# theEricMa/ScaleDreamer

Measured on AMD Instinct MI355X. Metric: ASD train steps/sec (64x64 render, SD2.1), higher is better.
Workload: dtype f32 renderer / f16 diffusion (f32 accumulate); 1 GPU; asd_sd_nerf: 1 view/GPU, 64x64 rays, 512 spp occgrid march, implicit-volume iNGP (16x2 hash grid 2^19, MLP 64), SD-2.1 UNet batch 5 (CFG+Perp-Neg+shifted t), VAE 512^2 fwd+bwd, AdamW; views_per_gpu=1, parallelism=dp1, diffusion_backend=hip, diffusion_weights=seeded random init (seed 1)

## Files before the change

scaledreamer_amd/csrc/gemm.hip:

```cpp
#include <stdlib.h>

#include "asd_common.h"
#include <map>
#include <atomic>
#include <mutex>
#include <cstring>
#include <iterator>

#include "gemm_tile.h"


template <int BM, int BN, int WM, int WN, bool CONV, int NST = 2, int KG = 1, bool LN = false>
__global__ __launch_bounds__(WM * WN * KG * 64) void gemm_f16_kernel(const asd_gemm_args p) {
    constexpr int NW = WM * WN;
    constexpr int TM = BM / WM / 16, TN = BN / WN / 16;
    constexpr int RB = 128;
    constexpr int A_BYTES = BM * RB, B_BYTES = BN * RB;
    constexpr int STAGE_BYTES = A_BYTES + B_BYTES;
    constexpr int ASLABS = BM / 8, TSLABS = (BM + BN) / 8;
    constexpr int SPW = (TSLABS + NW - 1) / NW;
    static_assert(BM % (WM * 16) == 0 && BN % (WN * 16) == 0, "wave tile must be a multiple of 16 x 16");
    static_assert(NST == 2 || TSLABS % NW == 0, "ring variants count their loads per wave: every wave must own the same number of slabs");
    static_assert(KG == 1 || NST == 2, "k-groups use the two-stage loop");
    extern __shared__ __attribute__((aligned(16))) char smem[];

    const int tid = threadIdx.x, lane = tid & 63;
    const int wave_all = __builtin_amdgcn_readfirstlane(tid >> 6);
    const int kg = KG > 1 ? wave_all / NW : 0;
    const int wave = wave_all - kg * NW;
    char* const gsm = smem + kg * (NST * STAGE_BYTES);
    const int wm = wave / WN, wn = wave % WN;
    const bool up3 = CONV && p.upsample == 3;
    const int up_mq = up3 ? p.M >> 2 : 1;
    const int tiles_pp = (up_mq + BM - 1) / BM;
    const int tiles_m = up3 ? 4 * tiles_pp : (p.M + BM - 1) / BM, tiles_n = (p.N + BN - 1) / BN;
    int item, tm_, tn_;
    if (!asd_xcd_item(blockIdx.x, tiles_m * tiles_n * p.split_k, item)) return;
    const int kz = item / (tiles_m * tiles_n);
    asd_grouped_tile(item - kz * tiles_m * tiles_n, tiles_m, tiles_n, p.group_m, p.group_n, tm_, tn_);
    const int parity = up3 ? tm_ / tiles_pp : 0;
    const int m0 = up3 ? parity * up_mq + (tm_ - parity * tiles_pp) * BM : tm_ * BM, n0 = tn_ * BN;
    const int m_lim = up3 ? (parity + 1) * up_mq : p.M;
    const int k_steps_total = (p.K + 63) / 64;
    const int k_per = (k_steps_total + p.split_k - 1) / p.split_k;
    const int ks0 = kz * k_per, ks1 = min(k_steps_total, ks0 + k_per);

// ... 246 lines not shown
#pragma unroll
            for (int s = 0; s < NST - 1; ++s)
                if (s < nk) issue(ks0 + s, s);
            int stage = 0, fill = NST - 1;
            for (int i = 0; i < nk; ++i) {
                ring_wait<SPW, NST - 2>(nk - 1 - i);
                __builtin_amdgcn_s_barrier();
                if (i + NST - 1 < nk) issue(ks0 + i + NST - 1, fill);
                compute(gsm + stage * STAGE_BYTES);
                stage = stage + 1 == NST ? 0 : stage + 1;
                fill = fill + 1 == NST ? 0 : fill + 1;
            }
        }
    } else {
    int k = ks0;
    while (k < ks1 && !live(k)) ++k;
    if (k < ks1) {
        issue(k, 0);
        for (int stage = 0;; stage ^= 1) {
            asm volatile("s_waitcnt vmcnt(0)" ::: "memory");
            __builtin_amdgcn_s_barrier();
            int kn = k + 1;
            while (kn < ks1 && !live(kn)) ++kn;
            if (kn < ks1) issue(kn, stage ^ 1);
            compute(gsm + stage * STAGE_BYTES);
            if (kn >= ks1) break;
            k = kn;
        }
    }
    }
    if constexpr (KG == 1) ln_extract();

    const int em = lane & 15, en = (lane >> 4) * 4;
    auto out_row = [&](int i) {
        const int m = m0 + wm * (BM / WM) + i * 16 + em;
        if (m >= m_lim) return -1;
        if (CONV && p.upsample == 3) {
            const int q = m - parity * up_mq, hwq = p.Hin * p.Win;
            const int bb = q / hwq, r = q - bb * hwq, y = r / p.Win, x = r - y * p.Win;
            return (bb * p.Hout + 2 * y + par_a) * p.Wout + 2 * x + par_b;
        }
        return m;
    };
    if (KG > 1 && kg != 0) {
        if (p.split_k == 1 && p.act != 2 && p.gn_partials != nullptr) {
            __syncthreads(); __syncthreads();
            __syncthreads();
        }
        return;
    }
    if (p.split_k > 1) {
        tile_epilogue<TM, TN>(p, acc, n0 + wn * (BN / WN), kz, m0, out_row, false, nullptr);
        return;
    }
    float ln_mean[LN ? TM : 1], ln_rstd[LN ? TM : 1];
    if constexpr (LN) {
        const float inv_k = 1.f / (float)p.K;
#pragma unroll
        for (int i = 0; i < TM; ++i) {
            ln_mean[i] = ls1[i] * inv_k;
            ln_rstd[i] = rsqrtf(fmaxf(ls2[i] * inv_k - ln_mean[i] * ln_mean[i], 0.f) + p.ln_eps);
            const int m = m0 + wm * (BM / WM) + i * 16 + em;
            if (p.ln_stats && n0 == 0 && wn == 0 && lane < 16 && m < p.M) { p.ln_stats[2 * m] = ln_mean[i]; p.ln_stats[2 * m + 1] = ln_rstd[i]; }
        }
    }
    if (p.act == 2) {
        if constexpr (TN % 2 == 0) {
#pragma unroll
            for (int i = 0; i < TM; ++i) {
                const int m = m0 + wm * (BM / WM) + i * 16 + em;
                if (m >= p.M) continue;
#pragma unroll
                for (int j = 0; j < TN; j += 2) {
                    const int n = n0 + wn * (BN / WN) + j * 16 + en;
                    if (n + 16 >= p.N) continue;
                    const half4 bx = *(const half4*)((const half_t*)p.bias + n), bg = *(const half4*)((const half_t*)p.bias + n + 16);
                    float va[4] = {acc[i][j][0], acc[i][j][1], acc[i][j][2], acc[i][j][3]};
                    float vg[4] = {acc[i][j + 1][0], acc[i][j + 1][1], acc[i][j + 1][2], acc[i][j + 1][3]};
                    if (p.ln_mode) {
                        ln_fold<4>(p, va, m, n, LN ? ln_mean[i] : 0.f, LN ? ln_rstd[i] : 0.f);
                        ln_fold<4>(p, vg, m, n + 16, LN ? ln_mean[i] : 0.f, LN ? ln_rstd[i] : 0.f);
                    }
                    half4 o;
#pragma unroll
                    for (int r = 0; r < 4; ++r)
// ... 270 lines not shown
                            acc[i][j] = __builtin_amdgcn_mfma_f32_16x16x32_f16(wb[kh][j], xa[kh][i], acc[i][j], 0, 0, 0);
            } else {
#pragma unroll
            for (int kh = 0; kh < 2; ++kh) {
                half8 xa[TM], wb[TN];
                const char* Ak = Ar + (((kh * 4 + fq) ^ csw) * 16);
#pragma unroll
                for (int i = 0; i < TM; ++i) xa[i] = *(const half8*)(Ak + i * WIN * RB);
#pragma unroll
                for (int j = 0; j < TN; ++j) wb[j] = *(const half8*)(Wt + fb0 + fswb[kh] + j * 16 * RB);
#pragma unroll
                for (int i = 0; i < TM; ++i)
#pragma unroll
                    for (int j = 0; j < TN; ++j)
                        acc[i][j] = __builtin_amdgcn_mfma_f32_16x16x32_f16(wb[j], xa[i], acc[i][j], 0, 0, 0);
            }
            }
        }
    }

    const bool gn = p.gn_partials != nullptr && p.split_k == 1;
    float* gn_lds = (float*)smem;
    if (gn) gn_tile_begin(gn_lds);
    tile_epilogue<TM, TN>(p, acc, n0 + wn * (BN / WN), kz, b * p.Hout * p.Wout,
                          [&](int i) { return (b * p.Hout + y0 + wm * 4 + i) * p.Wout + x0 + frow; }, gn, gn_lds);
    if (gn) gn_tile_end(p, gn_lds, tm * tiles_n + tn_);
}

__global__ __launch_bounds__(256) void splitk_epilogue_kernel(const asd_gemm_args p, int splits) {
    const size_t q = (size_t)blockIdx.x * 256 + threadIdx.x;
    const size_t total4 = (size_t)p.M * p.N / 4;
    if (q >= total4) return;
    const int m = (int)((q * 4) / p.N), n = (int)((q * 4) % p.N);
    floatx4 v = {0.f, 0.f, 0.f, 0.f};
    for (int s = 0; s < splits; ++s) {
        const floatx4 t = *(const floatx4*)(p.workspace + ((size_t)s * p.M + m) * p.N + n);
        v[0] += t[0]; v[1] += t[1]; v[2] += t[2]; v[3] += t[3];
    }
    if (p.bias) {
        const half4 b = *(const half4*)((const half_t*)p.bias + n);
        v[0] += (float)b[0]; v[1] += (float)b[1]; v[2] += (float)b[2]; v[3] += (float)b[3];
    }
    if (p.row_bias) {
        const half4 b = *(const half4*)((const half_t*)p.row_bias + (size_t)(m / p.rows_per_group) * p.ld_row_bias + n);
        v[0] += (float)b[0]; v[1] += (float)b[1]; v[2] += (float)b[2]; v[3] += (float)b[3];
    }
    if (p.act == 1) {
#pragma unroll
        for (int r = 0; r < 4; ++r) v[r] = asd_silu_fast(v[r]);
    }
    if (p.residual) {
        const half4 b = *(const half4*)((const half_t*)p.residual + (size_t)m * p.ldr + n);
        v[0] += (float)b[0]; v[1] += (float)b[1]; v[2] += (float)b[2]; v[3] += (float)b[3];
    }
    if (p.out_f32) {
        *(floatx4*)((float*)p.C + (size_t)m * p.ldc + n) = v;
    } else {
        half4 o = {(half_t)v[0], (half_t)v[1], (half_t)v[2], (half_t)v[3]};
        *(half4*)((half_t*)p.C + (size_t)m * p.ldc + n) = o;
    }
}

__global__ __launch_bounds__(256) void splitk_epilogue_gn_kernel(const asd_gemm_args p, int splits) {
    __shared__ float lds64[64];
    const int tiles_n = p.N / 64;
    const int mb = blockIdx.x / tiles_n, nb = blockIdx.x - mb * tiles_n;
    const int tx = threadIdx.x & 15, ty = threadIdx.x >> 4;
    const int n = nb * 64 + tx * 4;
    if (threadIdx.x < 64) lds64[threadIdx.x] = 0.f;
    __syncthreads();
    floatx4 cs = {0.f, 0.f, 0.f, 0.f}, cq = {0.f, 0.f, 0.f, 0.f};
    half4 bias = {0, 0, 0, 0};
    if (p.bias) bias = *(const half4*)((const half_t*)p.bias + n);
    floatx4 v[4];
    int mrow[4];
#pragma unroll
    for (int i = 0; i < 4; ++i) {
        v[i] = floatx4{0.f, 0.f, 0.f, 0.f};
        mrow[i] = min(mb * 64 + i * 16 + ty, p.M - 1);
    }
    for (int s = 0; s < splits; ++s) {
        floatx4 t[4];
#pragma unroll
        for (int i = 0; i < 4; ++i) t[i] = *(const floatx4*)(p.workspace + ((size_t)s * p.M + mrow[i]) * p.N + n);
#pragma unroll
        for (int i = 0; i < 4; ++i) { v[i][0] += t[i][0]; v[i][1] += t[i][1]; v[i][2] += t[i][2]; v[i][3] += t[i][3]; }
    }
#pragma unroll
    for (int i = 0; i < 4; ++i) {
        const int m = mb * 64 + i * 16 + ty;
        if (m >= p.M) continue;
        floatx4 w = v[i];
        w[0] += (float)bias[0]; w[1] += (float)bias[1]; w[2] += (float)bias[2]; w[3] += (float)bias[3];
        if (p.row_bias) {
            const half4 b = *(const half4*)((const half_t*)p.row_bias + (size_t)(m / p.rows_per_group) * p.ld_row_bias + n);
            w[0] += (float)b[0]; w[1] += (float)b[1]; w[2] += (float)b[2]; w[3] += (float)b[3];
        }
        if (p.act == 1) {
#pragma unroll
            for (int r = 0; r < 4; ++r) w[r] = asd_silu_fast(w[r]);
        }
        if (p.residual) {
            const half4 b = *(const half4*)((const half_t*)p.residual + (size_t)m * p.ldr + n);
            w[0] += (float)b[0]; w[1] += (float)b[1]; w[2] += (float)b[2]; w[3] += (float)b[3];
        }
        const half4 o = {(half_t)w[0], (half_t)w[1], (half_t)w[2], (half_t)w[3]};
        *(half4*)((half_t*)p.C + (size_t)m * p.ldc + n) = o;
#pragma unroll
        for (int r = 0; r < 4; ++r) { const float f = (float)o[r]; cs[r] += f; cq[r] = fmaf(f, f, cq[r]); }
    }
#pragma unroll
    for (int r = 0; r < 4; ++r) {
        const int g = (n + r) / p.gn_cg;
        atomicAdd(&lds64[2 * g], cs[r]);
        atomicAdd(&lds64[2 * g + 1], cq[r]);
    }
    __syncthreads();
    if (threadIdx.x < 64) p.gn_partials[(size_t)blockIdx.x * 64 + threadIdx.x] = lds64[threadIdx.x];
}

#define GNA_THREADS 1024
template <int NV>
__global__ __launch_bounds__(GNA_THREADS) void splitk_epilogue_gnapply_kernel(const asd_gemm_args p, int splits, float inv_cnt ) {
    __shared__ float red[2 * (GNA_THREADS / 64)];
    const int cg = p.gn_cg, g4 = cg >> 2, rows = p.gn_rows;
    const int b = blockIdx.x >> 5, g = blockIdx.x & 31;
    const int n0 = g * cg, total = rows * g4, tid = threadIdx.x;
    floatx4 v[NV];
    int mrow[NV], ncol[NV];
#pragma unroll
    for (int i = 0; i < NV; ++i) {
        const int e = min(tid + GNA_THREADS * i, total - 1);
        const int r = e / g4;
        mrow[i] = b * rows + r;
        ncol[i] = n0 + (e - r * g4) * 4;
        v[i] = floatx4{0.f, 0.f, 0.f, 0.f};
    }
    half4 bias[NV], rbias[NV], resid[NV];
#pragma unroll
    for (int i = 0; i < NV; ++i) {
        const int m = mrow[i], n = ncol[i];
        bias[i] = p.bias ? *(const half4*)((const half_t*)p.bias + n) : half4{0, 0, 0, 0};
        rbias[i] = p.row_bias ? *(const half4*)((const half_t*)p.row_bias + (size_t)(m / p.rows_per_group) * p.ld_row_bias + n) : half4{0, 0, 0, 0};
        resid[i] = p.residual ? *(const half4*)((const half_t*)p.residual + (size_t)m * p.ldr + n) : half4{0, 0, 0, 0};
    }
    for (int s = 0; s < splits; s += 4) {
        floatx4 t[4][NV];
#pragma unroll
        for (int u = 0; u < 4; ++u) {
            const int su = min(s + u, splits - 1);
#pragma unroll
// ... 54 lines not shown
#pragma unroll
        for (int r = 0; r < 4; ++r) {
            const float sa = rstd * (float)gm[r];
            float f = fmaf(v[i][r], sa, (float)bt[r] - mean * sa);
            if (p.gn_apply_silu) f = asd_silu_fast(f);
            o[r] = (half_t)f;
        }
        *(half4*)((half_t*)p.gn_apply_y + (size_t)m * p.N + n) = o;
    }
}

static int asd_gemm_gn_apply_nv(const asd_gemm_args* a) {
    if (!a->gn_apply || a->split_k <= 1 || a->partials_only || a->out_f32 || a->act == 2 || a->gn_bwd_x) return 0;
    if (a->gn_cg < 4 || a->gn_cg % 4 || a->N != 32 * a->gn_cg || a->gn_rows < 1 || a->M % a->gn_rows || a->ldc % 4) return 0;
    if (a->conv && a->upsample == 3) return 0;
    const int need = (a->gn_rows * (a->gn_cg / 4) + GNA_THREADS - 1) / GNA_THREADS;
    return need <= 1 ? 1 : need <= 3 ? 3 : 0;
}

static void asd_launch_splitk_epilogue(const asd_gemm_args* a, hipStream_t s) {
    const int nv = a->gn_apply_y ? asd_gemm_gn_apply_nv(a) : 0;
    if (nv > 0) {
        const dim3 grid((a->M / a->gn_rows) * 32);
        const float inv_cnt = 1.f / ((float)a->gn_rows * (float)a->gn_cg);
        if (nv == 1) hipLaunchKernelGGL(splitk_epilogue_gnapply_kernel<1>, grid, dim3(GNA_THREADS), 0, s, *a, a->split_k, inv_cnt);
        else hipLaunchKernelGGL(splitk_epilogue_gnapply_kernel<3>, grid, dim3(GNA_THREADS), 0, s, *a, a->split_k, inv_cnt);
        return;
    }
    const size_t total4 = (size_t)a->M * a->N / 4;
    if (a->gn_partials) hipLaunchKernelGGL(splitk_epilogue_gn_kernel, dim3((a->M / 64) * (a->N / 64)), dim3(256), 0, s, *a, a->split_k);
    else hipLaunchKernelGGL(splitk_epilogue_kernel, dim3(asd_div_up(total4, 256)), dim3(256), 0, s, *a, a->split_k);
}


struct asd_gemm_tile {
    int kind;
    int bm, bn, wm, wn;
    int nst, kg;
    int (*launch)(asd_gemm_args* a, hipStream_t s);
};

static void asd_pick_group(int tiles_m, int tiles_n, int bm, int bn, size_t lds, int* gm, int* gn) {
    const int conc = 32 * (2 * lds <= 160 * 1024 ? 2 : 1);
    int m = (int)lroundf(sqrtf((float)conc * (float)bn / (float)bm));
    m = m < 1 ? 1 : (m > tiles_m ? tiles_m : m);
    int n = conc / m;
    n = n < 1 ? 1 : (n > tiles_n ? tiles_n : n);
    if (n == tiles_n) { m = conc / n; m = m < 1 ? 1 : (m > tiles_m ? tiles_m : m); }
    *gm = m; *gn = n;
}

template <int BM, int BN, int WM, int WN, int NST, int KG>
static int asd_launch_plain(asd_gemm_args* a, hipStream_t s) {
    const int tiles = (a->conv && a->upsample == 3 ? 4 * asd_div_up(a->M / 4, BM) : asd_div_up(a->M, BM)) * asd_div_up(a->N, BN);
    const size_t lds = (size_t)NST * KG * (BM + BN) * 128;
    if (a->group_m < 1 || a->group_n < 1) asd_pick_group(asd_div_up(a->M, BM), asd_div_up(a->N, BN), BM, BN, lds, &a->group_m, &a->group_n);
    const dim3 grid(8 * asd_div_up(tiles * a->split_k, 8)), block(WM * WN * KG * 64);
    if (a->conv) asd_launch_lds<gemm_f16_kernel<BM, BN, WM, WN, true, NST, KG, false>>(grid, block, lds, s, *a);
    else if (a->ln_mode == 1) asd_launch_lds<gemm_f16_kernel<BM, BN, WM, WN, false, NST, KG, true>>(grid, block, lds, s, *a);
    else asd_launch_lds<gemm_f16_kernel<BM, BN, WM, WN, false, NST, KG, false>>(grid, block, lds, s, *a);
    return ASD_OK;
}

template <bool TWO, int BN, int NW>
static int asd_launch_window(asd_gemm_args* a, hipStream_t s) {
    const size_t lds = (size_t)(TWO ? 1 : 2) * (41 * 1024 + 2 * BN * 128);
    const int tiles_n = asd_div_up(a->N, BN);
    if (a->group_m < 1 || a->group_n < 1) asd_pick_group(a->M / 256, tiles_n, 256, BN, TWO ? (size_t)80 * 1024 : lds, &a->group_m, &a->group_n);
    const dim3 grid(8 * asd_div_up((a->M / 256) * tiles_n * a->split_k, 8)), block(NW * 64);
    if constexpr (TWO) asd_launch_lds<conv3x3_win2_kernel<BN, NW>>(grid, block, lds, s, *a);
    else asd_launch_lds<conv3x3_win_kernel<BN>>(grid, block, lds, s, *a);
    return ASD_OK;
}

size_t asd_conv_pp_lds_bytes(int tm, int tn);
template <int TM, int TN> void asd_conv_pp_launch(const asd_gemm_args* a, int blocks, hipStream_t s);
template <int TM, int TN>
static int asd_launch_pp(asd_gemm_args* a, hipStream_t s) {
    const int tiles_m = a->M / (64 * TM), tiles_n = a->N / (32 * TN);
    if (a->group_m < 1 || a->group_n < 1) asd_pick_group(tiles_m, tiles_n, 64 * TM, 32 * TN, asd_conv_pp_lds_bytes(TM, TN), &a->group_m, &a->group_n);
    asd_conv_pp_launch<TM, TN>(a, 8 * asd_div_up(tiles_m * tiles_n * a->split_k, 8), s);
    return ASD_OK;
}

int asd_conv_ws_launch(const asd_gemm_args* a, hipStream_t s);
static int asd_launch_ws(asd_gemm_args* a, hipStream_t s) {
    if (asd_conv_ws_launch(a, s) != ASD_OK) { asd_set_error("weight-streaming convolution: bad image count"); return ASD_ERR_ARG; }
    return ASD_OK;
}

template <int KIND, int BM, int BN, int WM, int WN, int NST, int KG>
static int asd_tile_launch(asd_gemm_args* a, hipStream_t s) {
    if constexpr (KIND == ASD_TILE_PLAIN) return asd_launch_plain<BM, BN, WM, WN, NST, KG>(a, s);
    else {
        static_assert(NST == 2 && KG == 1, "only the plain kernel has a ring depth and k-groups to choose");
        if constexpr (KIND == ASD_TILE_WIN) { static_assert(BM == 256 && WM * WN == 8, "window: 256 pixels, eight waves"); return asd_launch_window<false, BN, 8>(a, s); }
        else if constexpr (KIND == ASD_TILE_WIN2) { static_assert(BM == 256, "window: 256 pixels"); return asd_launch_window<true, BN, WM * WN>(a, s); }
        else if constexpr (KIND == ASD_TILE_PP) { static_assert(BM % 64 == 0 && BN % 32 == 0 && WM * WN == 8, "ping-pong: eight waves"); return asd_launch_pp<BM / 64, BN / 32>(a, s); }
        else { static_assert(KIND == ASD_TILE_WS && BM == 320 && BN == 64 && WM * WN == 4, "weight streaming: 5 x 64 rows, four waves"); return asd_launch_ws(a, s); }
    }
}
#define ASD_TILE(KIND, BM, BN, WM, WN, NST, KG) {ASD_TILE_##KIND, BM, BN, WM, WN, NST, KG, &asd_tile_launch<ASD_TILE_##KIND, BM, BN, WM, WN, NST, KG>}
static constexpr asd_gemm_tile asd_gemm_tiles[] = {
    ASD_TILE(PLAIN, 128, 64, 2, 2, 2, 1), ASD_TILE(PLAIN, 128, 128, 2, 2, 2, 1), ASD_TILE(PLAIN, 256, 64, 4, 2, 2, 1), ASD_TILE(PLAIN, 256, 128, 4, 2, 2, 1),
    ASD_TILE(PLAIN, 128, 320, 2, 4, 2, 1), ASD_TILE(PLAIN, 256, 256, 2, 4, 2, 1), ASD_TILE(PLAIN, 256, 320, 2, 4, 2, 1), ASD_TILE(PLAIN, 320, 128, 5, 2, 2, 1),
    ASD_TILE(WIN, 256, 64, 4, 2, 2, 1), ASD_TILE(WIN, 256, 128, 4, 2, 2, 1), ASD_TILE(WIN2, 256, 64, 4, 2, 2, 1), ASD_TILE(WIN2, 256, 128, 4, 2, 2, 1),
    ASD_TILE(PLAIN, 64, 64, 2, 2, 2, 1),
    ASD_TILE(WIN2, 256, 64, 4, 1, 2, 1), ASD_TILE(WIN2, 256, 128, 4, 1, 2, 1),
    ASD_TILE(PLAIN, 64, 64, 2, 2, 4, 1), ASD_TILE(PLAIN, 64, 64, 2, 2, 2, 2), ASD_TILE(PLAIN, 64, 64, 2, 2, 2, 4), ASD_TILE(PLAIN, 128, 64, 2, 2, 2, 2),
    ASD_TILE(PLAIN, 128, 128, 2, 2, 2, 2),
    ASD_TILE(PP, 512, 128, 4, 2, 2, 1), ASD_TILE(PP, 256, 256, 4, 2, 2, 1), ASD_TILE(PP, 256, 320, 4, 2, 2, 1), ASD_TILE(PP, 256, 128, 4, 2, 2, 1),
    ASD_TILE(PP, 256, 160, 4, 2, 2, 1),
    ASD_TILE(WS, 320, 64, 2, 2, 2, 1),
    ASD_TILE(PLAIN, 128, 64, 2, 2, 6, 1), ASD_TILE(PLAIN, 64, 64, 2, 2, 8, 1), ASD_TILE(PLAIN, 128, 128, 2, 2, 4, 1)};
#define ASD_GEMM_NCFG ((int)(sizeof(asd_gemm_tiles) / sizeof(asd_gemm_tiles[0])))

static constexpr bool asd_cfg_is(int cfg, int kind, int bm, int bn) {
    return asd_gemm_tiles[cfg].kind == kind && asd_gemm_tiles[cfg].bm == bm && asd_gemm_tiles[cfg].bn == bn;
}
static_assert(asd_cfg_is(ASD_CFG_128x64, ASD_TILE_PLAIN, 128, 64) && asd_cfg_is(ASD_CFG_128x128, ASD_TILE_PLAIN, 128, 128) &&
              asd_cfg_is(ASD_CFG_256x64, ASD_TILE_PLAIN, 256, 64) && asd_cfg_is(ASD_CFG_256x128, ASD_TILE_PLAIN, 256, 128) &&
              asd_cfg_is(ASD_CFG_256x256, ASD_TILE_PLAIN, 256, 256) && asd_cfg_is(ASD_CFG_320x128, ASD_TILE_PLAIN, 320, 128) &&
              asd_cfg_is(ASD_CFG_WIN_64, ASD_TILE_WIN, 256, 64) && asd_cfg_is(ASD_CFG_WIN_128, ASD_TILE_WIN, 256, 128) &&
              asd_cfg_is(ASD_CFG_WIN2_64, ASD_TILE_WIN2, 256, 64) && asd_cfg_is(ASD_CFG_WIN2_128, ASD_TILE_WIN2, 256, 128),
              "a named tile configuration moved");

static bool asd_cfg_is_plain(int cfg) { return asd_gemm_tiles[cfg].kind == ASD_TILE_PLAIN; }
static bool asd_cfg_is_pp(int cfg) { return asd_gemm_tiles[cfg].kind == ASD_TILE_PP; }
static bool asd_cfg_is_ws(int cfg) { return asd_gemm_tiles[cfg].kind == ASD_TILE_WS; }
static bool asd_cfg_is_window(int cfg) { return !asd_cfg_is_plain(cfg) && !asd_cfg_is_ws(cfg); }
static int asd_cfg_wave_n(int cfg) { return asd_gemm_tiles[cfg].bn / asd_gemm_tiles[cfg].wn; }
static bool asd_conv_ws_ok(const asd_gemm_args* a) {
    return a->conv && a->stride == 1 && a->pad == 1 && a->upsample == 0 && a->Hin == 8 && a->Win == 8 && a->Hout == 8 && a->Wout == 8 &&
           a->M % 64 == 0 && a->M / 64 <= 5 && a->N % 64 == 0 && a->split_k >= 2 && a->Cin % (32 * a->split_k) == 0 && !a->gn_bwd_x && !a->ln_mode;
}

static bool asd_conv_window_ok(const asd_gemm_args* a) {
    return a->conv && a->stride == 1 && a->pad == 1 && a->upsample == 0 && a->Cin % 64 == 0 && a->Hin == a->Hout &&
           a->Win == a->Wout && a->Hout % 16 == 0 && a->Wout % 16 == 0;
}

static bool asd_conv_pp_ok(const asd_gemm_args* a, int cfg) {
    return a->conv && a->stride == 1 && a->pad == 1 && a->upsample == 0 && a->Cin % 32 == 0 && a->Hin == a->Hout && a->Win == a->Wout &&
           a->Hout % 16 == 0 && a->Wout % 16 == 0 && a->Hout % (asd_gemm_tiles[cfg].bm / 16) == 0 && a->N % asd_gemm_tiles[cfg].bn == 0;
}
static int g_force_tile = -1;

static int asd_gemm_pick_tile(int M, int N, int K, int split) {
    const int ksteps = asd_div_up(asd_div_up(K, 64), split);
    double best = 1e300;
    int best_cfg = 1;
    for (int c = 0; c < ASD_GEMM_NCFG && asd_cfg_is_plain(c); ++c) {
        const int bm = asd_gemm_tiles[c].bm, bn = asd_gemm_tiles[c].bn;
        if (bn > 64 && N % bn != 0 && !(bn == 128 && N % 128 == 0)) continue;
        if (bn == 64 && N % 128 == 0) continue;
        const long long blocks = (long long)asd_div_up(M, bm) * asd_div_up(N, bn) * split;
        const double per_block = (double)ksteps * (bm + bn) + 6.0 * 64 + 0.02 * bm * bn;
        const double rounds = blocks >= 256 ? (double)blocks / 256.0 : 0.62 + 0.38 * (double)blocks / 256.0;
        const double cost = per_block * rounds;
        if (cost < best) { best = cost; best_cfg = c; }
    }
    return best_cfg;
}

struct asd_plan_key {
    int32_t M, N, K, conv, a, b, c, d, e;
    bool operator<(const asd_plan_key& o) const { return memcmp(this, &o, sizeof(*this)) < 0; }
};
struct asd_plan_val { int32_t tile, split; };
static std::map<asd_plan_key, asd_plan_val> g_plans;
static std::mutex g_plans_mu;
static std::atomic<uint64_t> g_plan_gen{1};

static asd_plan_key asd_plan_key_of(const asd_gemm_args* a) {
    asd_plan_key k;
    memset(&k, 0, sizeof(k));
    k.M = a->M; k.N = a->N; k.K = a->K; k.conv = a->conv ? 1 : 0;
    if (a->conv) { k.a = a->Hin; k.b = a->Cin; k.c = a->stride; k.d = a->upsample; k.e = a->pad; }
// ... 155 lines not shown
                      "GEGLU epilogue: N % 32 == 0, bias required, no conv / residual / row_bias / fp32 output / split-K");
    if (a->ln_mode) {
        ASD_CHECK_ARG((a->ln_mode == 1 || a->ln_mode == 2) && a->ln_sc && !a->out_f32, "LayerNorm fold: ln_mode 1 | 2, ln_sc required, fp16 output");
        ASD_CHECK_ARG(a->ln_mode == 1 || (a->ln_stats && a->N % 4 == 0), "LayerNorm fold, mode 2: the column statistics ln_stats[N][2] are required");
        ASD_CHECK_ARG(a->ln_mode == 2 || !a->conv, "LayerNorm fold, mode 1: plain GEMM only (the rows of A are the LayerNorm's rows)");
        if (a->split_k > 1) { a->split_k = 1; a->tile_cfg = 0; }
    }
    int cfg = asd_gemm_resolve_cfg(a);
    ASD_CHECK_ARG(a->act != 2 || (!asd_cfg_is_window(cfg) && asd_cfg_wave_n(cfg) % 32 == 0),
                  "GEGLU epilogue needs a tile whose per-wave width is a multiple of 32 columns");
    ASD_CHECK_ARG(asd_gemm_tiles[cfg].bn == 64 || a->N % asd_gemm_tiles[cfg].bn == 0 || (asd_gemm_tiles[cfg].bn == 128 && a->N % 4 == 0),
                  "tile configuration does not divide N");
    if (asd_gemm_gn_records_cfg(a, cfg, true) == 0) a->gn_partials = nullptr;
    {
        auto al16 = [](const void* q) { return ((uintptr_t)q & 15) == 0; };
        const int wave_n = asd_cfg_wave_n(cfg);
        a->wide_rows = wave_n % 32 == 0 && a->act != 2 && a->N % 8 == 0 && a->ldc % 8 == 0 && al16(a->C) && (!a->bias || al16(a->bias)) &&
                       (!a->row_bias || (al16(a->row_bias) && a->ld_row_bias % 8 == 0)) && (!a->residual || (al16(a->residual) && a->ldr % 8 == 0)) &&
                       !(a->gn_partials && a->gn_bwd_x);
    }
    static const bool trace = getenv("ASD_GEMM_TRACE") != nullptr;
    if (trace)
        fprintf(stderr, "ASD_GEMM %d %d %d conv=%d %d %d %d %d %d s=%d p=%d u=%d cfg=%d split=%d act=%d res=%d f32=%d gn=%d\n", a->M, a->N, a->K, a->conv, a->Hin,
                a->Win, a->Cin, a->Hout, a->Wout, a->stride, a->pad, a->upsample, cfg, a->split_k, a->act, a->residual != nullptr, a->out_f32,
                a->gn_partials ? (a->gn_bwd_x ? 2 : 1) : 0);
    if (asd_cfg_is_ws(cfg))
        ASD_CHECK_ARG(asd_conv_ws_ok(a), "weight-streaming convolution: 3x3 stride-1 pad-1 on <= 5 images of 8x8, N % 64 == 0, split_k >= 2, Cin % (32 split_k) == 0");
    if (asd_cfg_is_window(cfg)) {
        ASD_CHECK_ARG(asd_cfg_is_pp(cfg) ? asd_conv_pp_ok(a, cfg) : asd_conv_window_ok(a),
                      "window convolution needs a 3x3 stride-1 pad-1 conv with Cin % 64 == 0 (ping-pong: % 32) and H, W % 16 == 0");
        ASD_CHECK_ARG(a->split_k == 1 || a->split_k <= a->Cin / 64, "window convolution: split_k exceeds the channel chunks");
    }
    hipStream_t s = (hipStream_t)stream;
    const int rc = asd_gemm_tiles[cfg].launch(a, s);
    if (rc != ASD_OK) return rc;
    if (a->split_k > 1 && !a->partials_only) asd_launch_splitk_epilogue(a, s);
    ASD_LAUNCH_CHECK();
    return ASD_OK;
}


static int asd_tune_candidates(const asd_gemm_args* a, int (*out)[2], int max_out) {
    static const int sk_plain[] = {1, 2, 3, 4, 6, 8, 12, 16}, sk_win[] = {1, 2, 3, 4, 5, 6, 8, 10};
    const bool geglu = a->act == 2, window_ok = asd_conv_window_ok(a);
    int n = 0;
    for (int t = 0; t < ASD_GEMM_NCFG && n < max_out; ++t) {
        const int bm = asd_gemm_tiles[t].bm, bn = asd_gemm_tiles[t].bn;
        if (asd_cfg_is_ws(t)) {
            static const int sk_ws[] = {2, 4, 5, 8, 10, 16, 20};
            for (int sk : sk_ws) {
                asd_gemm_args q = *a;
                q.split_k = sk;
                if (!asd_conv_ws_ok(&q) || (a->N / 64) * sk > 512 || (a->N / 64) * sk < 64) continue;
                if (n < max_out) { out[n][0] = t + 1; out[n][1] = sk; ++n; }
            }
            continue;
        }
        if (asd_cfg_is_window(t)) {
            if (asd_cfg_is_pp(t) ? !asd_conv_pp_ok(a, t) : (!window_ok || (bn != 64 && a->N % bn != 0))) continue;
            const int tiles = (a->M / bm) * asd_div_up(a->N, bn);
            for (int sk : sk_win) {
                if (sk > 1 && (a->Cin / 64 < 2 * sk || tiles * sk > 1536)) continue;
                if (n < max_out) { out[n][0] = t + 1; out[n][1] = sk; ++n; }
            }
            continue;
        }
        if (bn != 64 && a->N % bn != 0) continue;
        const bool few = asd_gemm_tiles[t].nst > 2 || asd_gemm_tiles[t].kg > 1;
        if (few && ((a->conv && a->upsample == 2) || (long long)asd_div_up(a->M, bm) * asd_div_up(a->N, bn) > 512 || a->K < 512)) continue;
// ... 102 lines not shown
```

scaledreamer_amd/csrc/gemm_tile.h:

```cpp
#pragma once
#include "asd_common.h"

typedef _Float16 half_t;
typedef half_t half8 __attribute__((ext_vector_type(8)));
typedef half_t half4 __attribute__((ext_vector_type(4)));
typedef float floatx4 __attribute__((ext_vector_type(4)));

enum {
    ASD_CFG_128x64 = 0, ASD_CFG_128x128 = 1, ASD_CFG_256x64 = 2, ASD_CFG_256x128 = 3, ASD_CFG_256x256 = 5, ASD_CFG_320x128 = 7,
    ASD_CFG_WIN_64 = 8, ASD_CFG_WIN_128 = 9,
    ASD_CFG_WIN2_64 = 10, ASD_CFG_WIN2_128 = 11
};

#define GLOBAL_AS __attribute__((address_space(1)))
#define LDS_AS __attribute__((address_space(3)))

__device__ __forceinline__ float gelu_erf(float x) {
    const float z = fabsf(x) * 0.70710678118654752440f;
    const float t = __builtin_amdgcn_rcpf(fmaf(0.3275911f, z, 1.f));
    float poly = fmaf(1.061405429f, t, -1.453152027f);
    poly = fmaf(poly, t, 1.421413741f);
    poly = fmaf(poly, t, -0.284496736f);
    poly = fmaf(poly, t, 0.254829592f);
    const float tail = poly * t * __builtin_amdgcn_exp2f(-1.44269504088896340736f * z * z);
// ... 133 lines not shown
__device__ __forceinline__ void gemm_store8(const asd_gemm_args& p, floatx4& lo, floatx4& hi, int m, int n) {
    float v[8] = {lo[0], lo[1], lo[2], lo[3], hi[0], hi[1], hi[2], hi[3]};
    if (p.bias) {
        const half8 b = *(const half8*)((const half_t*)p.bias + n);
#pragma unroll
        for (int k = 0; k < 8; ++k) v[k] += (float)b[k];
    }
    if (p.row_bias) {
        const half8 b = *(const half8*)((const half_t*)p.row_bias + (size_t)(m / p.rows_per_group) * p.ld_row_bias + n);
#pragma unroll
        for (int k = 0; k < 8; ++k) v[k] += (float)b[k];
    }
    if (p.act == 1) {
#pragma unroll
        for (int k = 0; k < 8; ++k) v[k] = asd_silu_fast(v[k]);
    }
    if (p.residual) {
        const half8 b = *(const half8*)((const half_t*)p.residual + (size_t)m * p.ldr + n);
#pragma unroll
        for (int k = 0; k < 8; ++k) v[k] += (float)b[k];
    }
    if (p.out_f32) {
        float* dst = (float*)p.C + (size_t)m * p.ldc + n;
        *(floatx4*)dst = floatx4{v[0], v[1], v[2], v[3]};
        *(floatx4*)(dst + 4) = floatx4{v[4], v[5], v[6], v[7]};
        lo = floatx4{v[0], v[1], v[2], v[3]}; hi = floatx4{v[4], v[5], v[6], v[7]};
        return;
    }
    const half8 o = {(half_t)v[0], (half_t)v[1], (half_t)v[2], (half_t)v[3], (half_t)v[4], (half_t)v[5], (half_t)v[6], (half_t)v[7]};
    *(half8*)((half_t*)p.C + (size_t)m * p.ldc + n) = o;
    lo = floatx4{(float)o[0], (float)o[1], (float)o[2], (float)o[3]}; hi = floatx4{(float)o[4], (float)o[5], (float)o[6], (float)o[7]};
}

template <int TM, int TN, typename RowFn>
__device__ __forceinline__ void tile_epilogue(const asd_gemm_args& p, floatx4 (&acc)[TM][TN], int nb, int kz, int row0, RowFn row, bool gn, float* gn_lds,
                                              const float* ln_mean = nullptr, const float* ln_rstd = nullptr) {
    const int g = (threadIdx.x & 63) >> 4;
    if constexpr (TN % 2 == 0) {
        if (p.wide_rows) {
#pragma unroll
            for (int s2 = 0; s2 < TN / 2; ++s2) {
                const int n = nb + s2 * 32 + g * 8;
                floatx4 cs0 = {0.f, 0.f, 0.f, 0.f}, cq0 = cs0, cs1 = cs0, cq1 = cs0;
#pragma unroll
                for (int i = 0; i < TM; ++i) {
                    const int m = row(i);
                    if (m < 0 || n >= p.N) continue;
                    if (p.split_k > 1) {
                        float* dst = p.workspace + ((size_t)kz * p.M + m) * p.N + n;
                        *(floatx4*)dst = acc[i][2 * s2];
                        *(floatx4*)(dst + 4) = acc[i][2 * s2 + 1];
                    } else {
                        floatx4 lo = acc[i][2 * s2], hi = acc[i][2 * s2 + 1];
                        if (p.ln_mode) {
                            float v8[8] = {lo[0], lo[1], lo[2], lo[3], hi[0], hi[1], hi[2], hi[3]};
                            ln_fold<8>(p, v8, m, n, ln_mean ? ln_mean[i] : 0.f, ln_rstd ? ln_rstd[i] : 0.f);
                            lo = floatx4{v8[0], v8[1], v8[2], v8[3]}; hi = floatx4{v8[4], v8[5], v8[6], v8[7]};
                        }
                        gemm_store8(p, lo, hi, m, n);
                        if (gn) {
#pragma unroll
                            for (int r = 0; r < 4; ++r) {
                                cs0[r] += lo[r]; cq0[r] = fmaf(lo[r], lo[r], cq0[r]);
                                cs1[r] += hi[r]; cq1[r] = fmaf(hi[r], hi[r], cq1[r]);
                            }
                        }
                    }
                }
                if (gn) { gn_tile_flush(gn_lds, cs0, cq0, n, p.N, p.gn_cg); gn_tile_flush(gn_lds, cs1, cq1, n + 4, p.N, p.gn_cg); }
            }
            return;
        }
    }
#pragma unroll
    for (int j = 0; j < TN; ++j) {
        const int n = nb + j * 16 + g * 4;
        floatx4 cs = {0.f, 0.f, 0.f, 0.f}, cq = {0.f, 0.f, 0.f, 0.f};
        GnCol gc;
        if (gn) gn_col_load(p, row0, n, gc);
#pragma unroll
        for (int i = 0; i < TM; ++i) {
            const int m = row(i);
            if (m < 0 || n >= p.N) continue;
            if (p.split_k > 1) *(floatx4*)(p.workspace + ((size_t)kz * p.M + m) * p.N + n) = acc[i][j];
            else {
                floatx4 a4 = acc[i][j];
                if (p.ln_mode) {
                    float v4[4] = {a4[0], a4[1], a4[2], a4[3]};
                    ln_fold<4>(p, v4, m, n, ln_mean ? ln_mean[i] : 0.f, ln_rstd ? ln_rstd[i] : 0.f);
                    a4 = floatx4{v4[0], v4[1], v4[2], v4[3]};
                }
                const floatx4 o = gemm_store4(p, a4, m, n);
                if (gn) gn_tile_accum(p, gc, o, m, n, cs, cq);
            }
        }
        if (gn) gn_tile_flush(gn_lds, cs, cq, n, p.N, p.gn_cg);
    }
}

template <int PER, int MAX>
__device__ __forceinline__ void ring_wait(int ahead) {
    if constexpr (MAX <= 0) {
        asm volatile("s_waitcnt vmcnt(0)" ::: "memory");
    } else {
        if (ahead >= MAX) asm volatile("s_waitcnt vmcnt(%0)" ::"n"(MAX * PER) : "memory");
        else ring_wait<PER, MAX - 1>(ahead);
    }
}
```

Baseline: 70.58 steps/s.

## Fuse split-K reduction into GEMM via last-arriver tile counters

Small split-K GEMMs now do their own reduction. Each K-slice writes its partial slab with write-through stores and bumps a per-tile atomic counter, and the last block to arrive sums all slices and runs the epilogue. This removes the separate split-K epilogue kernel launch and its extra round trip for the affected GEMMs. It adds a pooled counter buffer that rotates through 64 slots, memory fences and atomics. It also carries a risk that counters collide if more than 64 GEMMs are in flight at once. The standalone epilogue kernels are refactored onto shared helpers, with the reduction loop unrolled to two slices at a time.

Result: no change. 70.37 steps/s (-0.3%).

```diff
diff --git a/scaledreamer_amd/csrc/gemm.hip b/scaledreamer_amd/csrc/gemm.hip
--- a/scaledreamer_amd/csrc/gemm.hip
+++ b/scaledreamer_amd/csrc/gemm.hip
@@ -11,7 +11,7 @@
 
 
 template <int BM, int BN, int WM, int WN, bool CONV, int NST = 2, int KG = 1, bool LN = false>
-__global__ __launch_bounds__(WM * WN * KG * 64) void gemm_f16_kernel(const asd_gemm_args p) {
+__global__ __launch_bounds__(WM * WN * KG * 64) void gemm_f16_kernel(const asd_gemm_args p, unsigned* const sk_cnt ) {
     constexpr int NW = WM * WN;
     constexpr int TM = BM / WM / 16, TN = BN / WN / 16;
     constexpr int RB = 128;
@@ -324,8 +324,8 @@
     if constexpr (KG == 1) ln_extract();
 
     const int em = lane & 15, en = (lane >> 4) * 4;
-    auto out_row = [&](int i) {
-        const int m = m0 + wm * (BM / WM) + i * 16 + em;
+    auto tile_row = [&p, m0, m_lim, parity, up_mq, par_a, par_b](int r) {
+        const int m = m0 + r;
         if (m >= m_lim) return -1;
         if (CONV && p.upsample == 3) {
             const int q = m - parity * up_mq, hwq = p.Hin * p.Win;
@@ -334,6 +334,7 @@
         }
         return m;
     };
+    auto out_row = [&](int i) { return tile_row(wm * (BM / WM) + i * 16 + em); };
     if (KG > 1 && kg != 0) {
         if (p.split_k == 1 && p.act != 2 && p.gn_partials != nullptr) {
             __syncthreads(); __syncthreads();
@@ -342,7 +343,14 @@
         return;
     }
     if (p.split_k > 1) {
-        tile_epilogue<TM, TN>(p, acc, n0 + wn * (BN / WN), kz, m0, out_row, false, nullptr);
+        tile_epilogue<TM, TN>(p, acc, n0 + wn * (BN / WN), kz, m0, out_row, false, nullptr, nullptr, nullptr, sk_cnt != nullptr);
+        if constexpr (!LN) {
+            unsigned* const cnt = sk_cnt ? sk_cnt + (item - kz * tiles_m * tiles_n) : nullptr;
+            if (cnt && splitk_arrive(cnt, p.split_k, smem)) {
+                splitk_reduce_range<BN / 4, NW * 64>(p, p.split_k, BM, n0, tile_row, tid);
+                splitk_leave(cnt);
+            }
+        }
         return;
     }
     float ln_mean[LN ? TM : 1], ln_rstd[LN ? TM : 1];
@@ -679,91 +687,17 @@
     const size_t total4 = (size_t)p.M * p.N / 4;
     if (q >= total4) return;
     const int m = (int)((q * 4) / p.N), n = (int)((q * 4) % p.N);
-    floatx4 v = {0.f, 0.f, 0.f, 0.f};
-    for (int s = 0; s < splits; ++s) {
-        const floatx4 t = *(const floatx4*)(p.workspace + ((size_t)s * p.M + m) * p.N + n);
-        v[0] += t[0]; v[1] += t[1]; v[2] += t[2]; v[3] += t[3];
-    }
-    if (p.bias) {
-        const half4 b = *(const half4*)((const half_t*)p.bias + n);
-        v[0] += (float)b[0]; v[1] += (float)b[1]; v[2] += (float)b[2]; v[3] += (float)b[3];
-    }
-    if (p.row_bias) {
-        const half4 b = *(const half4*)((const half_t*)p.row_bias + (size_t)(m / p.rows_per_group) * p.ld_row_bias + n);
-        v[0] += (float)b[0]; v[1] += (float)b[1]; v[2] += (float)b[2]; v[3] += (float)b[3];
-    }
-    if (p.act == 1) {
-#pragma unroll
-        for (int r = 0; r < 4; ++r) v[r] = asd_silu_fast(v[r]);
-    }
-    if (p.residual) {
-        const half4 b = *(const half4*)((const half_t*)p.residual + (size_t)m * p.ldr + n);
-        v[0] += (float)b[0]; v[1] += (float)b[1]; v[2] += (float)b[2]; v[3] += (float)b[3];
-    }
-    if (p.out_f32) {
-        *(floatx4*)((float*)p.C + (size_t)m * p.ldc + n) = v;
-    } else {
-        half4 o = {(half_t)v[0], (half_t)v[1], (half_t)v[2], (half_t)v[3]};
-        *(half4*)((half_t*)p.C + (size_t)m * p.ldc + n) = o;
-    }
+    const float* const src[1] = {p.workspace + q * 4};
+    floatx4 v[1];
+    splitk_sum<1>(p, splits, src, v);
+    gemm_store4(p, v[0], m, n);
 }
 
 __global__ __launch_bounds__(256) void splitk_epilogue_gn_kernel(const asd_gemm_args p, int splits) {
     __shared__ float lds64[64];
     const int tiles_n = p.N / 64;
     const int mb = blockIdx.x / tiles_n, nb = blockIdx.x - mb * tiles_n;
-    const int tx = threadIdx.x & 15, ty = threadIdx.x >> 4;
-    const int n = nb * 64 + tx * 4;
-    if (threadIdx.x < 64) lds64[threadIdx.x] = 0.f;
-    __syncthreads();
-    floatx4 cs = {0.f, 0.f, 0.f, 0.f}, cq = {0.f, 0.f, 0.f, 0.f};
-    half4 bias = {0, 0, 0, 0};
-    if (p.bias) bias = *(const half4*)((const half_t*)p.bias + n);
-    floatx4 v[4];
-    int mrow[4];
-#pragma unroll
-    for (int i = 0; i < 4; ++i) {
-        v[i] = floatx4{0.f, 0.f, 0.f, 0.f};
-        mrow[i] = min(mb * 64 + i * 16 + ty, p.M - 1);
-    }
-    for (int s = 0; s < splits; ++s) {
-        floatx4 t[4];
-#pragma unroll
-        for (int i = 0; i < 4; ++i) t[i] = *(const floatx4*)(p.workspace + ((size_t)s * p.M + mrow[i]) * p.N + n);
-#pragma unroll
-        for (int i = 0; i < 4; ++i) { v[i][0] += t[i][0]; v[i][1] += t[i][1]; v[i][2] += t[i][2]; v[i][3] += t[i][3]; }
-    }
-#pragma unroll
-    for (int i = 0; i < 4; ++i) {
-        const int m = mb * 64 + i * 16 + ty;
-        if (m >= p.M) continue;
-        floatx4 w = v[i];
-        w[0] += (float)bias[0]; w[1] += (float)bias[1]; w[2] += (float)bias[2]; w[3] += (float)bias[3];
-        if (p.row_bias) {
-            const half4 b = *(const half4*)((const half_t*)p.row_bias + (size_t)(m / p.rows_per_group) * p.ld_row_bias + n);
-            w[0] += (float)b[0]; w[1] += (float)b[1]; w[2] += (float)b[2]; w[3] += (float)b[3];
-        }
-        if (p.act == 1) {
-#pragma unroll
-            for (int r = 0; r < 4; ++r) w[r] = asd_silu_fast(w[r]);
-        }
-        if (p.residual) {
-            const half4 b = *(const half4*)((const half_t*)p.residual + (size_t)m * p.ldr + n);
-            w[0] += (float)b[0]; w[1] += (float)b[1]; w[2] += (float)b[2]; w[3] += (float)b[3];
-        }
-        const half4 o = {(half_t)w[0], (half_t)w[1], (half_t)w[2], (half_t)w[3]};
-        *(half4*)((half_t*)p.C + (size_t)m * p.ldc + n) = o;
-#pragma unroll
-        for (int r = 0; r < 4; ++r) { const float f = (float)o[r]; cs[r] += f; cq[r] = fmaf(f, f, cq[r]); }
-    }
-#pragma unroll
-    for (int r = 0; r < 4; ++r) {
-        const int g = (n + r) / p.gn_cg;
-        atomicAdd(&lds64[2 * g], cs[r]);
-        atomicAdd(&lds64[2 * g + 1], cq[r]);
-    }
-    __syncthreads();
-    if (threadIdx.x < 64) p.gn_partials[(size_t)blockIdx.x * 64 + threadIdx.x] = lds64[threadIdx.x];
+    splitk_reduce_gn_block<256>(p, splits, mb, nb, lds64, threadIdx.x);
 }
 
 #define GNA_THREADS 1024
@@ -884,12 +818,34 @@
     else hipLaunchKernelGGL(splitk_epilogue_kernel, dim3(asd_div_up(total4, 256)), dim3(256), 0, s, *a, a->split_k);
 }
 
+#define ASD_SPLITK_SLOTS 64
+#define ASD_SPLITK_SLOT_TILES 2048
+static unsigned* asd_splitk_slot(hipStream_t s) {
+    static std::mutex mu;
+    static unsigned* pools[64] = {nullptr};
+    static unsigned next = 0;
+    int dev = 0;
+    (void)hipGetDevice(&dev);
+    if (dev < 0 || dev >= 64) return nullptr;
+    std::lock_guard<std::mutex> lock(mu);
+    if (!pools[dev]) {
+        hipStreamCaptureStatus st = hipStreamCaptureStatusNone;
+        if (hipStreamIsCapturing(s, &st) != hipSuccess || st != hipStreamCaptureStatusNone) { (void)hipGetLastError(); return nullptr; }
+        const size_t bytes = (size_t)ASD_SPLITK_SLOTS * ASD_SPLITK_SLOT_TILES * sizeof(unsigned);
+        void* q = nullptr;
+        if (hipMalloc(&q, bytes) != hipSuccess) { (void)hipGetLastError(); return nullptr; }
+        if (hipMemset(q, 0, bytes) != hipSuccess || hipDeviceSynchronize() != hipSuccess) { (void)hipGetLastError(); (void)hipFree(q); return nullptr; }
+        pools[dev] = (unsigned*)q;
+    }
+    return pools[dev] + (size_t)(next++ % ASD_SPLITK_SLOTS) * ASD_SPLITK_SLOT_TILES;
+}
+
 
 struct asd_gemm_tile {
     int kind;
     int bm, bn, wm, wn;
     int nst, kg;
-    int (*launch)(asd_gemm_args* a, hipStream_t s);
+    int (*launch)(asd_gemm_args* a, hipStream_t s, unsigned* sk_cnt);
 };
 
 static void asd_pick_group(int tiles_m, int tiles_n, int bm, int bn, size_t lds, int* gm, int* gn) {
@@ -903,14 +859,14 @@
 }
 
 template <int BM, int BN, int WM, int WN, int NST, int KG>
-static int asd_launch_plain(asd_gemm_args* a, hipStream_t s) {
+static int asd_launch_plain(asd_gemm_args* a, hipStream_t s, unsigned* sk_cnt) {
     const int tiles = (a->conv && a->upsample == 3 ? 4 * asd_div_up(a->M / 4, BM) : asd_div_up(a->M, BM)) * asd_div_up(a->N, BN);
     const size_t lds = (size_t)NST * KG * (BM + BN) * 128;
     if (a->group_m < 1 || a->group_n < 1) asd_pick_group(asd_div_up(a->M, BM), asd_div_up(a->N, BN), BM, BN, lds, &a->group_m, &a->group_n);
     const dim3 grid(8 * asd_div_up(tiles * a->split_k, 8)), block(WM * WN * KG * 64);
-    if (a->conv) asd_launch_lds<gemm_f16_kernel<BM, BN, WM, WN, true, NST, KG, false>>(grid, block, lds, s, *a);
-    else if (a->ln_mode == 1) asd_launch_lds<gemm_f16_kernel<BM, BN, WM, WN, false, NST, KG, true>>(grid, block, lds, s, *a);
-    else asd_launch_lds<gemm_f16_kernel<BM, BN, WM, WN, false, NST, KG, false>>(grid, block, lds, s, *a);
+    if (a->conv) asd_launch_lds<gemm_f16_kernel<BM, BN, WM, WN, true, NST, KG, false>>(grid, block, lds, s, *a, sk_cnt);
+    else if (a->ln_mode == 1) asd_launch_lds<gemm_f16_kernel<BM, BN, WM, WN, false, NST, KG, true>>(grid, block, lds, s, *a, sk_cnt);
+    else asd_launch_lds<gemm_f16_kernel<BM, BN, WM, WN, false, NST, KG, false>>(grid, block, lds, s, *a, sk_cnt);
     return ASD_OK;
 }
 
@@ -942,8 +898,8 @@
 }
 
 template <int KIND, int BM, int BN, int WM, int WN, int NST, int KG>
-static int asd_tile_launch(asd_gemm_args* a, hipStream_t s) {
-    if constexpr (KIND == ASD_TILE_PLAIN) return asd_launch_plain<BM, BN, WM, WN, NST, KG>(a, s);
+static int asd_tile_launch(asd_gemm_args* a, hipStream_t s, unsigned* sk_cnt) {
+    if constexpr (KIND == ASD_TILE_PLAIN) return asd_launch_plain<BM, BN, WM, WN, NST, KG>(a, s, sk_cnt);
     else {
         static_assert(NST == 2 && KG == 1, "only the plain kernel has a ring depth and k-groups to choose");
         if constexpr (KIND == ASD_TILE_WIN) { static_assert(BM == 256 && WM * WN == 8, "window: 256 pixels, eight waves"); return asd_launch_window<false, BN, 8>(a, s); }
@@ -996,6 +952,17 @@
     return a->conv && a->stride == 1 && a->pad == 1 && a->upsample == 0 && a->Cin % 32 == 0 && a->Hin == a->Hout && a->Win == a->Wout &&
            a->Hout % 16 == 0 && a->Wout % 16 == 0 && a->Hout % (asd_gemm_tiles[cfg].bm / 16) == 0 && a->N % asd_gemm_tiles[cfg].bn == 0;
 }
+#define ASD_SPLITK_IN_LAUNCH_MAX_BYTES (16 * 1024)
+static bool asd_splitk_in_launch(const asd_gemm_args* a, int cfg) {
+    const asd_gemm_tile& t = asd_gemm_tiles[cfg];
+    if (a->split_k <= 1 || a->partials_only || t.kind != ASD_TILE_PLAIN || a->ln_mode) return false;
+    if (a->gn_partials || (a->gn_apply_y && asd_gemm_gn_apply_nv(a) > 0)) return false;
+    const bool up3 = a->conv && a->upsample == 3;
+    const long long tiles_m = up3 ? 4 * asd_div_up(a->M / 4, t.bm) : asd_div_up(a->M, t.bm);
+    if (tiles_m * asd_div_up(a->N, t.bn) > ASD_SPLITK_SLOT_TILES) return false;
+    return (long long)a->split_k * (a->M < t.bm ? a->M : t.bm) * t.bn * 4 <= ASD_SPLITK_IN_LAUNCH_MAX_BYTES;
+}
+
 static int g_force_tile = -1;
 
 static int asd_gemm_pick_tile(int M, int N, int K, int split) {
@@ -1217,9 +1184,10 @@
         ASD_CHECK_ARG(a->split_k == 1 || a->split_k <= a->Cin / 64, "window convolution: split_k exceeds the channel chunks");
     }
     hipStream_t s = (hipStream_t)stream;
-    const int rc = asd_gemm_tiles[cfg].launch(a, s);
+    unsigned* const sk_cnt = asd_splitk_in_launch(a, cfg) ? asd_splitk_slot(s) : nullptr;
+    const int rc = asd_gemm_tiles[cfg].launch(a, s, sk_cnt);
     if (rc != ASD_OK) return rc;
-    if (a->split_k > 1 && !a->partials_only) asd_launch_splitk_epilogue(a, s);
+    if (a->split_k > 1 && !a->partials_only && !sk_cnt) asd_launch_splitk_epilogue(a, s);
     ASD_LAUNCH_CHECK();
     return ASD_OK;
 }
diff --git a/scaledreamer_amd/csrc/gemm_tile.h b/scaledreamer_amd/csrc/gemm_tile.h
--- a/scaledreamer_amd/csrc/gemm_tile.h
+++ b/scaledreamer_amd/csrc/gemm_tile.h
@@ -189,9 +189,14 @@
     lo = floatx4{(float)o[0], (float)o[1], (float)o[2], (float)o[3]}; hi = floatx4{(float)o[4], (float)o[5], (float)o[6], (float)o[7]};
 }
 
+__device__ __forceinline__ void slab_store16(float* dst, const floatx4& v, bool wt) {
+    if (wt) asm volatile("global_store_dwordx4 %0, %1, off sc1\n\ts_nop 1" ::"v"(dst), "v"(v) : "memory");
+    else *(floatx4*)dst = v;
+}
+
 template <int TM, int TN, typename RowFn>
 __device__ __forceinline__ void tile_epilogue(const asd_gemm_args& p, floatx4 (&acc)[TM][TN], int nb, int kz, int row0, RowFn row, bool gn, float* gn_lds,
-                                              const float* ln_mean = nullptr, const float* ln_rstd = nullptr) {
+                                              const float* ln_mean = nullptr, const float* ln_rstd = nullptr, bool sk_wt = false) {
     const int g = (threadIdx.x & 63) >> 4;
     if constexpr (TN % 2 == 0) {
         if (p.wide_rows) {
@@ -205,8 +210,8 @@
                     if (m < 0 || n >= p.N) continue;
                     if (p.split_k > 1) {
                         float* dst = p.workspace + ((size_t)kz * p.M + m) * p.N + n;
-                        *(floatx4*)dst = acc[i][2 * s2];
-                        *(floatx4*)(dst + 4) = acc[i][2 * s2 + 1];
+                        slab_store16(dst, acc[i][2 * s2], sk_wt);
+                        slab_store16(dst + 4, acc[i][2 * s2 + 1], sk_wt);
                     } else {
                         floatx4 lo = acc[i][2 * s2], hi = acc[i][2 * s2 + 1];
                         if (p.ln_mode) {
@@ -239,7 +244,7 @@
         for (int i = 0; i < TM; ++i) {
             const int m = row(i);
             if (m < 0 || n >= p.N) continue;
-            if (p.split_k > 1) *(floatx4*)(p.workspace + ((size_t)kz * p.M + m) * p.N + n) = acc[i][j];
+            if (p.split_k > 1) slab_store16(p.workspace + ((size_t)kz * p.M + m) * p.N + n, acc[i][j], sk_wt);
             else {
                 floatx4 a4 = acc[i][j];
                 if (p.ln_mode) {
@@ -255,6 +260,99 @@
     }
 }
 
+template <int NR>
+__device__ __forceinline__ void splitk_sum(const asd_gemm_args& p, int splits, const float* const (&src)[NR], floatx4 (&v)[NR]) {
+    const size_t slab = (size_t)p.M * p.N;
+#pragma unroll
+    for (int i = 0; i < NR; ++i) v[i] = floatx4{0.f, 0.f, 0.f, 0.f};
+    for (int s = 0; s < splits; s += 2) {
+        const bool two = s + 1 < splits;
+        floatx4 t0[NR], t1[NR];
+#pragma unroll
+        for (int i = 0; i < NR; ++i) t0[i] = *(const floatx4*)(src[i] + (size_t)s * slab);
+#pragma unroll
+        for (int i = 0; i < NR; ++i) t1[i] = *(const floatx4*)(src[i] + (size_t)(two ? s + 1 : s) * slab);
+#pragma unroll
+        for (int i = 0; i < NR; ++i) { v[i][0] += t0[i][0]; v[i][1] += t0[i][1]; v[i][2] += t0[i][2]; v[i][3] += t0[i][3]; }
+        if (two) {
+#pragma unroll
+            for (int i = 0; i < NR; ++i) { v[i][0] += t1[i][0]; v[i][1] += t1[i][1]; v[i][2] += t1[i][2]; v[i][3] += t1[i][3]; }
+        }
+    }
+}
+
+template <int COLS4, int NTH, typename RowFn>
+__device__ __forceinline__ void splitk_reduce_range(const asd_gemm_args& p, int splits, int rows, int n0, RowFn row, int tid) {
+    constexpr int U = 4;
+    const int total = rows * COLS4;
+    for (int e0 = tid; e0 < total; e0 += U * NTH) {
+        int m[U], n[U];
+        const float* src[U];
+#pragma unroll
+        for (int u = 0; u < U; ++u) {
+            const int e = e0 + u * NTH, r = e / COLS4;
+            m[u] = e < total ? row(r) : -1;
+            n[u] = n0 + (e - r * COLS4) * 4;
+            if (n[u] >= p.N) m[u] = -1;
+            src[u] = m[u] >= 0 ? p.workspace + (size_t)m[u] * p.N + n[u] : p.workspace;
+        }
+        floatx4 v[U];
+        splitk_sum<U>(p, splits, src, v);
+#pragma unroll
+        for (int u = 0; u < U; ++u)
+            if (m[u] >= 0) gemm_store4(p, v[u], m[u], n[u]);
+    }
+}
+
+template <int NTH>
+__device__ __forceinline__ void splitk_reduce_gn_block(const asd_gemm_args& p, int splits, int mb, int nb, float* lds64, int tid) {
+    constexpr int RP = NTH / 16, NR = 64 / RP;
+    static_assert(NTH % 16 == 0 && 64 % RP == 0, "a pass is whole rows of 16 float4 columns");
+    const int tx = tid & 15, ty = tid >> 4;
+    const int n = nb * 64 + tx * 4;
+    if (tid < 64) lds64[tid] = 0.f;
+    __syncthreads();
+    int m[NR];
+    const float* src[NR];
+#pragma unroll
+    for (int i = 0; i < NR; ++i) { m[i] = min(mb * 64 + i * RP + ty, p.M - 1); src[i] = p.workspace + (size_t)m[i] * p.N + n; }
+    floatx4 v[NR];
+    splitk_sum<NR>(p, splits, src, v);
+    floatx4 cs = {0.f, 0.f, 0.f, 0.f}, cq = {0.f, 0.f, 0.f, 0.f};
+#pragma unroll
+    for (int i = 0; i < NR; ++i) {
+        if (mb * 64 + i * RP + ty >= p.M) continue;
+        const floatx4 o = gemm_store4(p, v[i], m[i], n);
+#pragma unroll
+        for (int r = 0; r < 4; ++r) { cs[r] += o[r]; cq[r] = fmaf(o[r], o[r], cq[r]); }
+    }
+#pragma unroll
+    for (int r = 0; r < 4; ++r) {
+        const int g = (n + r) / p.gn_cg;
+        atomicAdd(&lds64[2 * g], cs[r]);
+        atomicAdd(&lds64[2 * g + 1], cq[r]);
+    }
+    __syncthreads();
+    if (tid < 64) p.gn_partials[((size_t)mb * (p.N / 64) + nb) * 64 + tid] = lds64[tid];
+}
+
+__device__ __forceinline__ bool splitk_arrive(unsigned* cnt, int splits, char* smem) {
+    asm volatile("s_waitcnt vmcnt(0)" ::: "memory");
+    __syncthreads();
+    if (threadIdx.x == 0) *(volatile unsigned*)smem = __hip_atomic_fetch_add(cnt, 1u, __ATOMIC_RELAXED, __HIP_MEMORY_SCOPE_AGENT);
+    __syncthreads();
+    if (*(volatile unsigned*)smem != (unsigned)(splits - 1)) return false;
+    if (threadIdx.x == 0) {
+        __builtin_amdgcn_fence(__ATOMIC_ACQUIRE, "agent");
+        asm volatile("s_waitcnt vmcnt(0)" ::: "memory");
+    }
+    __syncthreads();
+    return true;
+}
+__device__ __forceinline__ void splitk_leave(unsigned* cnt) {
+    if (threadIdx.x == 0) __hip_atomic_store(cnt, 0u, __ATOMIC_RELAXED, __HIP_MEMORY_SCOPE_AGENT);
+}
+
 template <int PER, int MAX>
 __device__ __forceinline__ void ring_wait(int ahead) {
     if constexpr (MAX <= 0) {
```
